# kmaninis/OSVOS-PyTorch

Measured on AMD Instinct MI355X. Metric: frames/sec (fwd+bwd) OSVOS-VGG16 854x480 per GPU; mask IoU vs ref, higher is better.
Workload: dtype f32 (3x bf16-split operands on MFMA, f32 accumulate); 1 GPU; 854x480 batch=1 online fine-tune loop (train_online.py), fused-head loss, nAveGrad=5, SGD 8-group, fp32x3, frame resident in HBM; global_batch=1, parallelism=dp1, grad_allreduce=none, rccl_ranks_seen=1

## Files before the change

osvos-pytorch_amd/csrc/wgrad_f32x3.hip:

```cpp
#include "common.h"
#include "kernels.h"
#include "h2split.h"

namespace {

typedef __bf16 bf16x8_t __attribute__((ext_vector_type(8)));
typedef __bf16 bf16x2_t __attribute__((ext_vector_type(2)));
typedef unsigned int u32x4 __attribute__((ext_vector_type(4)));
typedef short s16x4 __attribute__((ext_vector_type(4)));
typedef short s16x8 __attribute__((ext_vector_type(8)));
typedef __attribute__((address_space(3))) s16x4 lds_s16x4;

constexpr int PW = 16;

template <int PH_, int WAVES_, int S16_ = 0>
struct G3 {
  static constexpr int PH = PH_, WAVES = WAVES_, NT = 64 * WAVES_, S16 = S16_;
  static constexpr int BCO = S16_ ? 32 : 16 * WAVES_;
  static constexpr int BCI = S16_ ? 128 : 64;
  static constexpr int XOCT = BCI / 8;
  static constexpr int DYP = BCO * 2 + 64, XP = BCI * 2 + 64;
  static constexpr int PPIX = PW * PH, HW_ = PW + 2, XPIX = (PH + 2) * HW_;
  static constexpr int DY_B = PPIX * DYP, X_B = XPIX * XP;
  static constexpr int DOCT = BCO / 8;
  static constexpr int DY_ITEMS = PPIX * DOCT, X_ITEMS = XPIX * XOCT;
  static constexpr int DPG = NT / DOCT, XPG = NT / XOCT;
  static constexpr int NDY = (DY_ITEMS + NT - 1) / NT, NX = (X_ITEMS + NT - 1) / NT, NIT = NDY + NX;
  static constexpr int NST = 3 * PH;
  static constexpr int NB = WAVES_ == 8 ? 1 : 2;
  static constexpr size_t LDS = (size_t)3 * (DY_B + X_B);
  static_assert(NIT <= NST, "one staged item per stage must cover the patch");
  static_assert(LDS <= 160 * 1024, "tiles exceed the LDS of a CU");
};

struct W3Args {
  const void* x;
  const void* dy;
  float* slab;
  float* bslab;
  int N, H, W, Cin_s, Cout, Cout_s;
  int npx, npy, npatches, per_split, nco_t, nci_t;
  int map;
};

__device__ inline unsigned cvt2w(float a, float b) {
  bf16x2_t h;
  h[0] = (__bf16)a;
  h[1] = (__bf16)b;
  return __builtin_bit_cast(unsigned, h);
}
__device__ inline void split2w(float a, float b, unsigned& p0, unsigned& p1, unsigned& p2) {
  p0 = cvt2w(a, b);
  float ra = a - __uint_as_float(p0 << 16), rb = b - __uint_as_float(p0 & 0xffff0000u);
  p1 = cvt2w(ra, rb);
  ra -= __uint_as_float(p1 << 16);
  rb -= __uint_as_float(p1 & 0xffff0000u);
  p2 = cvt2w(ra, rb);
}
__device__ inline void split8w(const u32x4& lo, const u32x4& hi, u32x4& p0, u32x4& p1, u32x4& p2) {
  const f32x4 a = __builtin_bit_cast(f32x4, lo), b = __builtin_bit_cast(f32x4, hi);
  unsigned q0[4], q1[4], q2[4];
  split2w(a[0], a[1], q0[0], q1[0], q2[0]);
  split2w(a[2], a[3], q0[1], q1[1], q2[1]);
  split2w(b[0], b[1], q0[2], q1[2], q2[2]);
  split2w(b[2], b[3], q0[3], q1[3], q2[3]);
  p0 = u32x4{q0[0], q0[1], q0[2], q0[3]};
  p1 = u32x4{q1[0], q1[1], q1[2], q1[3]};
  p2 = u32x4{q2[0], q2[1], q2[2], q2[3]};
}

template <int NDS, int NVM, int NM = 18, int I = 0>
__device__ __forceinline__ void stage_groups() {
  if constexpr (I < NM) {
    __builtin_amdgcn_sched_group_barrier(0x008, 1, 0);
    constexpr int nds = (NDS * (I + 1)) / NM - (NDS * I) / NM, nvm = (NVM * (I + 1)) / NM - (NVM * I) / NM;
    if constexpr (nds > 0) __builtin_amdgcn_sched_group_barrier(0x100, nds, 0);
    if constexpr (nvm > 0) __builtin_amdgcn_sched_group_barrier(0x020, nvm, 0);
    __builtin_amdgcn_sched_group_barrier(0x006, 3, 0);
    stage_groups<NDS, NVM, NM, I + 1>();
  }
}

template <int PH, int WAVES, int S16 = 0, int ILV = 0, int NP = 3, int HP = 0, int OA = 0>
__global__ __launch_bounds__(64 * WAVES) void wgrad_f32x3_kernel(W3Args a) {
  static_assert(HP == 0 || NP == 2, "h2: two pieces");
  using G = G3<PH, WAVES, S16>;
  constexpr int NT = G::NT, BCO = G::BCO, BCI = G::BCI;
  extern __shared__ __attribute__((aligned(16))) char smem[];
  char* dYs = smem;
  char* Xs = smem + 3 * G::DY_B;
  const int tid = threadIdx.x, lane = tid & 63, wave = tid >> 6;
  const int wc = S16 ? 0 : wave >> 1, wi = S16 ? wave : wave & 1;
  constexpr unsigned OOB = 0x80000000u;

  int id = blockIdx.x;
  if (a.map == 1) id = (id & 7) * (gridDim.x >> 3) + (id >> 3);
  const int cit = id % a.nci_t;
  id /= a.nci_t;
  const int cot = id % a.nco_t;
  const int split = id / a.nco_t;
  const int co0 = cot * BCO, ci0 = cit * BCI;
  const int p_begin = split * a.per_split, p_end = min(p_begin + a.per_split, a.npatches);

  const int doct = tid % G::DOCT, dpg = tid / G::DOCT;
  const int xoct = tid % G::XOCT, xpg = tid / G::XOCT;
  const bool dy_ch_ok = co0 + 8 * doct < a.Cout, x_ch_ok = ci0 + 8 * xoct < a.Cin_s;
  u32x4 rdy[G::NDY][2], rx[G::NX][2];
  float bsum[8] = {0.f, 0.f, 0.f, 0.f, 0.f, 0.f, 0.f, 0.f};
  const bool want_bias = a.bslab != nullptr && cit == 0;
  const int img_dy_bytes = a.H * a.W * a.Cout_s * 4, img_x_bytes = a.H * a.W * a.Cin_s * 4;

  constexpr int DEADCOL = 0x40000000;
  unsigned dy_inv[G::NDY], x_inv[G::NX];
  unsigned dy_col[G::NDY], x_col[G::NX];
  if constexpr (OA == 0) {
#pragma unroll
    for (int it = 0; it < G::NDY; ++it) {
      const int p = dpg + G::DPG * it, py = p / PW, pxx = p - py * PW;
      const bool ok = dy_ch_ok && (G::DY_ITEMS % NT == 0 || p < G::PPIX);
      dy_inv[it] = (unsigned)(((py * a.W + pxx) * a.Cout_s + co0 + 8 * doct) * 4);
      dy_col[it] = (unsigned)(ok ? pxx : DEADCOL);
    }
#pragma unroll
    for (int j = 0; j < G::NX; ++j) {
      const int hp = xpg + G::XPG * j, hy = hp / G::HW_, hx = hp - hy * G::HW_;
      const bool ok = x_ch_ok && hp < G::XPIX;
      x_inv[j] = (unsigned)((((hy - 1) * a.W + hx - 1) * a.Cin_s + ci0 + 8 * xoct) * 4);
      x_col[j] = (unsigned)(ok ? hx - 1 : DEADCOL);
    }
  }

  struct Patch { __amdgpu_buffer_rsrc_t drs, xrs; int x0, y0; unsigned dorg, xorg; };
  auto locate = [&](int p, bool live) -> Patch {
    const int px = p % a.npx;
    int t = p / a.npx;
    const int py = t % a.npy;
    const int n = live ? t / a.npy : 0;
    Patch q;
    q.x0 = live ? px * PW : 0x40000000;
    q.y0 = py * PH;
    const unsigned org = (unsigned)(q.y0 * a.W + (live ? px * PW : 0));
    q.dorg = org * (unsigned)a.Cout_s * 4u;
    q.xorg = org * (unsigned)a.Cin_s * 4u;
    q.drs = __builtin_amdgcn_make_buffer_rsrc(const_cast<char*>(reinterpret_cast<const char*>(a.dy)) + (size_t)n * img_dy_bytes, 0, img_dy_bytes, 0x00020000);
    q.xrs = __builtin_amdgcn_make_buffer_rsrc(const_cast<char*>(reinterpret_cast<const char*>(a.x)) + (size_t)n * img_x_bytes, 0, img_x_bytes, 0x00020000);
    return q;
  };
  auto issue = [&](const Patch& q, int it) {
    if (it < G::NDY) {
      unsigned off;
      if constexpr (OA == 0) {
        off = (unsigned)q.x0 + dy_col[it] < (unsigned)a.W ? q.dorg + dy_inv[it] : OOB;
      } else {
        const int p = dpg + G::DPG * it, py = p / PW, pxx = p - py * PW;
        const bool ok = dy_ch_ok && (G::DY_ITEMS % NT == 0 || p < G::PPIX) && q.x0 + pxx < a.W;
        off = ok ? (unsigned)((((q.y0 + py) * a.W + q.x0 + pxx) * a.Cout_s + co0 + 8 * doct) * 4) : OOB;
      }
      rdy[it][0] = __builtin_amdgcn_raw_buffer_load_b128(q.drs, off, 0, 0);
      rdy[it][1] = __builtin_amdgcn_raw_buffer_load_b128(q.drs, off + 16u, 0, 0);
    } else if (it < G::NIT) {
      const int j = it - G::NDY;
      unsigned off;
      if constexpr (OA == 0) {
        off = (unsigned)q.x0 + x_col[j] < (unsigned)a.W ? q.xorg + x_inv[j] : OOB;
      } else {
        const int hp = xpg + G::XPG * j, hy = hp / G::HW_, hx = hp - hy * G::HW_;
        const bool ok = x_ch_ok && hp < G::XPIX && (unsigned)(q.x0 - 1 + hx) < (unsigned)a.W;
        off = ok ? (unsigned)((((q.y0 - 1 + hy) * a.W + q.x0 - 1 + hx) * a.Cin_s + ci0 + 8 * xoct) * 4) : OOB;
      }
      rx[j][0] = __builtin_amdgcn_raw_buffer_load_b128(q.xrs, off, 0, 0);
      rx[j][1] = __builtin_amdgcn_raw_buffer_load_b128(q.xrs, off + 16u, 0, 0);
    }
  };
  int h2_ed = kH2NoScale, h2_ex = kH2NoScale;
  float h2_sd = 1.f, h2_sx = 1.f;
  unsigned* const h2_mx = reinterpret_cast<unsigned*>(smem + G::LDS - 128);
  static_assert(HP == 0 || (G::X_B >= 128 && WAVES <= 8), "h2: exchange slots");
  auto store_patch = [&]() {
#pragma unroll
    for (int i = 0; i < G::NDY; ++i) {
      u32x4 p0, p1, p2;
      if (want_bias) {
        const f32x4 lo = __builtin_bit_cast(f32x4, rdy[i][0]), hi = __builtin_bit_cast(f32x4, rdy[i][1]);
#pragma unroll
        for (int c = 0; c < 4; ++c) { bsum[c] += lo[c]; bsum[4 + c] += hi[c]; }
      }
      if constexpr (HP != 0) h2_split8(rdy[i][0], rdy[i][1], h2_sd, p0, p1);
      else split8w(rdy[i][0], rdy[i][1], p0, p1, p2);
      const int p = dpg + G::DPG * i;
      if (G::DY_ITEMS % NT == 0 || p < G::PPIX) {
        char* d = dYs + p * G::DYP + doct * 16;
        *reinterpret_cast<u32x4*>(d) = p0;
        *reinterpret_cast<u32x4*>(d + G::DY_B) = p1;
        if constexpr (NP == 3) *reinterpret_cast<u32x4*>(d + 2 * G::DY_B) = p2;
      }
    }
#pragma unroll
    for (int j = 0; j < G::NX; ++j) {
      u32x4 p0, p1, p2;
      if constexpr (HP != 0) h2_split8(rx[j][0], rx[j][1], h2_sx, p0, p1);
      else split8w(rx[j][0], rx[j][1], p0, p1, p2);
      const int hp = xpg + G::XPG * j;
      if (G::X_ITEMS % NT == 0 || hp < G::XPIX) {
        char* d = Xs + hp * G::XP + xoct * 16;
        *reinterpret_cast<u32x4*>(d) = p0;
        *reinterpret_cast<u32x4*>(d + G::X_B) = p1;
        if constexpr (NP == 3) *reinterpret_cast<u32x4*>(d + 2 * G::X_B) = p2;
      }
    }
  };

  f32x16 acc[9];
#pragma unroll
  for (int t = 0; t < 9; ++t)
#pragma unroll
    for (int r = 0; r < 16; ++r) acc[t][r] = 0.f;

  const int fi = lane & 15, fg = (lane >> 4) & 1, lh = lane >> 5;
  const char* a_base = dYs + (8 * lh + (fi >> 2)) * G::DYP + (32 * wc + 16 * fg + 4 * (fi & 3)) * 2;
  const char* b_base = Xs + (8 * lh + (fi >> 2)) * G::XP + (32 * wi + 16 * fg + 4 * (fi & 3)) * 2;
  auto tr8 = [&](const char* p, int pitch) -> s16x8 {
    const s16x4 lo = __builtin_amdgcn_ds_read_tr16_b64_v4i16((lds_s16x4*)(p));
    const s16x4 hi = __builtin_amdgcn_ds_read_tr16_b64_v4i16((lds_s16x4*)(p + 4 * pitch));
    return __builtin_shufflevector(lo, hi, 0, 1, 2, 3, 4, 5, 6, 7);
  };

  {
    const Patch q = locate(p_begin, p_begin < p_end);
#pragma unroll
    for (int it = 0; it < G::NIT; ++it) issue(q, it);
  }
  for (int p = p_begin; p < p_end; ++p) {
    if constexpr (HP != 0) {
      unsigned md = 0, mxx = 0;
#pragma unroll
      for (int i = 0; i < G::NDY; ++i) md = h2_amax8(rdy[i][0], rdy[i][1], md);
#pragma unroll
      for (int j = 0; j < G::NX; ++j) mxx = h2_amax8(rx[j][0], rx[j][1], mxx);
      md = h2_wave_max(md);
      mxx = h2_wave_max(mxx);
      if (lane == 0) { h2_mx[(p & 1) * 16 + wave] = md; h2_mx[(p & 1) * 16 + 8 + wave] = mxx; }
    }
    __syncthreads();
    if constexpr (HP != 0) {
      const uint4* q = reinterpret_cast<const uint4*>(h2_mx) + (p & 1) * 4;
      const uint4 d0 = q[0], d1 = q[1], x0 = q[2], x1 = q[3];
      unsigned md = max(max(d0.x, d0.y), max(d0.z, d0.w)), mxx = max(max(x0.x, x0.y), max(x0.z, x0.w));
      if (WAVES == 8) { md = max(md, max(max(d1.x, d1.y), max(d1.z, d1.w))); mxx = max(mxx, max(max(x1.x, x1.y), max(x1.z, x1.w))); }
      const int ed = h2_exp(__builtin_amdgcn_readfirstlane(md)), ex = h2_exp(__builtin_amdgcn_readfirstlane(mxx));
      const int nd = ed < h2_ed ? ed : h2_ed, nx_ = ex < h2_ex ? ex : h2_ex;
      if (nd != h2_ed || nx_ != h2_ex) {
        const int dl = (h2_ed == kH2NoScale ? 0 : nd - h2_ed) + (h2_ex == kH2NoScale ? 0 : nx_ - h2_ex);
        if (dl != 0) {
#pragma unroll
          for (int t = 0; t < 9; ++t)
#pragma unroll
            for (int r = 0; r < 16; ++r) acc[t][r] = __builtin_ldexpf(acc[t][r], dl);
        }
        h2_ed = nd; h2_ex = nx_;
        h2_sd = h2_pow2(nd); h2_sx = h2_pow2(nx_);
      }
    }
    store_patch();
    __syncthreads();
    const Patch nx = locate(p + 1, p + 1 < p_end);
    constexpr int NB = G::NB;
    s16x8 af[NB][3], bfr[NB][3][3];
    auto lda = [&](int ks) {
#pragma unroll
      for (int pc = 0; pc < NP; ++pc) af[ks & (NB - 1)][pc] = tr8(a_base + pc * G::DY_B + ks * PW * G::DYP, G::DYP);
    };
    auto ldb = [&](int st) {
      const int ks = st / 3, r = st % 3;
#pragma unroll
      for (int pc = 0; pc < NP; ++pc)
#pragma unroll
        for (int s = 0; s < 3; ++s) bfr[st & (NB - 1)][pc][s] = tr8(b_base + pc * G::X_B + ((ks + r) * G::HW_ + s) * G::XP, G::XP);
    };
    if constexpr (NB == 2) {
      lda(0);
      ldb(0);
    }
#pragma unroll
    for (int st = 0; st < G::NST; ++st) {
      const int ks = st / 3, r = st % 3;
      if constexpr (NB == 2) {
        if (st + 1 < G::NST) {
          if (r == 2) lda(ks + 1);
          ldb(st + 1);
        }
      } else {
        if (r == 0) lda(ks);
        ldb(st);
      }
      issue(nx, st);
      if constexpr (ILV == 0) __builtin_amdgcn_sched_barrier(0);
      constexpr int NPROD = NP == 3 ? 6 : 3;
      constexpr int PX[6] = {NP == 3 ? 2 : 1, 0, NP == 3 ? 1 : 0, 1, 0, 0};
      constexpr int PD[6] = {0, NP == 3 ? 2 : 1, NP == 3 ? 1 : 0, 0, 1, 0};
#pragma unroll
      for (int t = 0; t < NPROD; ++t)
#pragma unroll
        for (int s = 0; s < 3; ++s)
          if constexpr (HP != 0)
            acc[r * 3 + s] = __builtin_amdgcn_mfma_f32_32x32x16_f16(__builtin_bit_cast(f16x8_t, bfr[st & (NB - 1)][PX[t]][s]),
                                                                   __builtin_bit_cast(f16x8_t, af[ks & (NB - 1)][PD[t]]), acc[r * 3 + s], 0, 0, 0);
          else
            acc[r * 3 + s] = __builtin_amdgcn_mfma_f32_32x32x16_bf16(__builtin_bit_cast(bf16x8_t, bfr[st & (NB - 1)][PX[t]][s]),
                                                                    __builtin_bit_cast(bf16x8_t, af[ks & (NB - 1)][PD[t]]), acc[r * 3 + s], 0, 0, 0);
      if constexpr (ILV != 0) {
        constexpr int V = 2;
        const bool last = st + 1 >= G::NST, wide = r == 2, vm = st < G::NIT;
        constexpr int NM = 3 * NPROD, DN = 6 * NP, DW = 8 * NP;
        if (last) { if (vm) stage_groups<0, V, NM>(); else stage_groups<0, 0, NM>(); }
        else if (wide) { if (vm) stage_groups<DW, V, NM>(); else stage_groups<DW, 0, NM>(); }
        else { if (vm) stage_groups<DN, V, NM>(); else stage_groups<DN, 0, NM>(); }
      }
      __builtin_amdgcn_sched_barrier(0);
    }
  }
  __syncthreads();
  if constexpr (HP != 0) {
    const int dl = (h2_ed == kH2NoScale || h2_ex == kH2NoScale) ? 0 : -(h2_ed + h2_ex);
#pragma unroll
    for (int t = 0; t < 9; ++t)
#pragma unroll
      for (int r = 0; r < 16; ++r) acc[t][r] = __builtin_ldexpf(acc[t][r], dl);
  }

  {
    const int li = lane & 31;
    const size_t slab_elems = (size_t)9 * a.Cout * a.Cin_s;
    const __amdgpu_buffer_rsrc_t srs = __builtin_amdgcn_make_buffer_rsrc(a.slab + (size_t)split * slab_elems, 0, (int)(slab_elems * 4), 0x00020000);
    const int co = co0 + wc * 32 + li;
    const int cib = ci0 + wi * 32 + 4 * lh;
    const unsigned row = co < a.Cout ? (unsigned)(co * a.Cin_s) * 4u : OOB;
    const unsigned tap_stride = (unsigned)(a.Cout * a.Cin_s) * 4u;
#pragma unroll
    for (int t = 0; t < 9; ++t)
#pragma unroll
      for (int q = 0; q < 4; ++q) {
        const int ci = cib + 8 * q;
        const unsigned off = ci < a.Cin_s ? row + (unsigned)t * tap_stride + (unsigned)ci * 4u : OOB;
        const f32x4 v = {acc[t][4 * q], acc[t][4 * q + 1], acc[t][4 * q + 2], acc[t][4 * q + 3]};
        __builtin_amdgcn_raw_buffer_store_b128(__builtin_bit_cast(u32x4, v), srs, off, 0, 0);
      }
  }
  if (want_bias) {
    float* red = reinterpret_cast<float*>(smem);
#pragma unroll
    for (int c = 0; c < 8; ++c) red[dpg * BCO + doct * 8 + c] = bsum[c];
    __syncthreads();
    if (tid < BCO) {
      float sum = 0.f;
      for (int g = 0; g < G::DPG; ++g) sum += red[g * BCO + tid];
      if (co0 + tid < a.Cout) a.bslab[(size_t)split * a.Cout + co0 + tid] = sum;
    }
  }
}

struct W3Plan {
  int ph, waves, bco, nco_t, nci_t, npx, npy, npatches, nsplit, per_split;
  size_t slab_floats, bslab_floats;
};

W3Plan make_plan3(int N, int H, int W, int Cin_s, int Cout) {
  W3Plan p;
  if (Cout == 16) {
    p.waves = 4; p.bco = 32; p.ph = 4;
    p.nco_t = 1;
    p.nci_t = ceil_div(Cin_s, 128);
    p.npx = ceil_div(W, PW);
    p.npy = ceil_div(H, p.ph);
    p.npatches = N * p.npx * p.npy;
    int want = ceil_div(256, p.nci_t);
    const int max_split = p.npatches / 2 > 0 ? p.npatches / 2 : 1;
    if (want > max_split) want = max_split;
    p.per_split = ceil_div(p.npatches, want);
    p.nsplit = ceil_div(p.npatches, p.per_split);
    p.slab_floats = (size_t)p.nsplit * 9 * Cout * Cin_s;
    p.bslab_floats = (size_t)p.nsplit * Cout;
    return p;
  }
  p.waves = 4;
  p.bco = 16 * p.waves;
  p.ph = (ceil_div(H, 6) * 6 <= ceil_div(H, 4) * 4) ? 6 : 4;
  p.nco_t = ceil_div(Cout, p.bco);
  p.nci_t = ceil_div(Cin_s, 64);
  p.npx = ceil_div(W, PW);
  p.npy = ceil_div(H, p.ph);
  p.npatches = N * p.npx * p.npy;
  int want = ceil_div(256, p.nco_t * p.nci_t);
  const int max_split = p.npatches / 2 > 0 ? p.npatches / 2 : 1;
  if (want > max_split) want = max_split;
  if (want > 256) want = 256;
  p.per_split = ceil_div(p.npatches, want);
  p.nsplit = ceil_div(p.npatches, p.per_split);
  p.slab_floats = (size_t)p.nsplit * 9 * Cout * Cin_s;
  p.bslab_floats = (size_t)p.nsplit * Cout;
  return p;
}

int block_map3(long blocks) {
  OSVOS_ENV_INT(map_env, "OSVOS_WGRAD_MAP", 1);
  return (map_env == 1 && blocks % 8 == 0) ? 1 : 0;
}

template <int PH, int WAVES, int S16 = 0, int ILV = 0, int NP = 3, int HP = 0, int OA = 0>
int launch3(const W3Args& a, long blocks, hipStream_t stream) {
  constexpr size_t lds = G3<PH, WAVES, S16>::LDS;
  if (int rc = osvos_set_dyn_lds_once<&wgrad_f32x3_kernel<PH, WAVES, S16, ILV, NP, HP, OA>>(lds)) return rc;
  hipLaunchKernelGGL((wgrad_f32x3_kernel<PH, WAVES, S16, ILV, NP, HP, OA>), dim3((unsigned)blocks), dim3(64 * WAVES), lds, stream, a);
  OSVOS_LAUNCH_CHECK();
  return 0;
}

}

bool osvos_wgrad_f32x3_applicable(int Cin, int Cin_s, int Cout, int Cout_s) {
  return Cin == Cin_s && Cin_s % 64 == 0 && Cout % 64 == 0 && Cout_s % 4 == 0;
}
bool osvos_wgrad_f32x3_skinny_applicable(int Cin, int Cin_s, int Cout, int Cout_s) {
  return Cout == 16 && Cout_s == 16 && Cin == Cin_s && Cin_s % 128 == 0;
}

size_t osvos_wgrad_f32x3_ws_bytes(int N, int H, int W, int Cin_s, int Cout) {
  if (Cout == 16 && Cin_s % 128 == 0) {
    const W3Plan p = make_plan3(N, H, W, Cin_s, Cout);
    return align_up((p.slab_floats + p.bslab_floats) * sizeof(float), 256);
  }
  if (Cin_s % 64 != 0 || Cout % 64 != 0) return 0;
  const W3Plan p = make_plan3(N, H, W, Cin_s, Cout);
  return align_up((p.slab_floats + p.bslab_floats) * sizeof(float), 256);
}

int osvos_wgrad_f32x3_plan(int N, int H, int W, int Cin_s, int Cout, int* out) {
  OSVOS_ARG_CHECK(osvos_wgrad_f32x3_applicable(Cin_s, Cin_s, Cout, Cout) || osvos_wgrad_f32x3_skinny_applicable(Cin_s, Cin_s, Cout, Cout),
                  "wgrad_wide_plan: no f32x3 weight-gradient kernel for Cin %d Cout %d", Cin_s, Cout);
  const W3Plan p = make_plan3(N, H, W, Cin_s, Cout);
  const long blocks = (long)p.nsplit * p.nco_t * p.nci_t;
  out[0] = PW; out[1] = p.ph; out[2] = p.npx; out[3] = p.npy; out[4] = p.npatches; out[5] = p.per_split; out[6] = p.nsplit;
  out[7] = p.nco_t; out[8] = p.nci_t; out[9] = (int)blocks; out[10] = block_map3(blocks); out[11] = 0;
  return 0;
}

int osvos_conv3x3_wgrad_f32x3(const WgradCall& c) {
  float *const dw = c.dw, *const db = c.db;
  void* const ws = c.ws; hipStream_t stream = c.stream;
  const int N = c.N, H = c.H, W = c.W, Cin = c.Cin, Cin_s = c.Cin_s, Cout = c.Cout, Cout_s = c.Cout_s, accumulate = c.accumulate;
  OSVOS_ARG_CHECK(c.x && c.dy && ws && dw, "wgrad f32x3: null pointer");
  OSVOS_ARG_CHECK(N > 0 && H > 0 && W > 0, "wgrad f32x3: bad shape");
  const bool skinny = Cout == 16 && Cout_s == 16 && Cin == Cin_s && Cin_s % 128 == 0;
  OSVOS_ARG_CHECK(skinny || osvos_wgrad_f32x3_applicable(Cin, Cin_s, Cout, Cout_s),
                  "wgrad f32x3: unsupported shape (Cin %d/%d Cout %d/%d)", Cin, Cin_s, Cout, Cout_s);
  OSVOS_ARG_CHECK((long)H * W * Cin_s < (1L << 28) && (long)H * W * Cout_s < (1L << 28), "wgrad f32x3: image too large for 31-bit byte offsets");
  OSVOS_ARG_CHECK(!c.x_bf16 && !c.dy_bf16, "wgrad f32x3: fp32 tensors only");
  const W3Plan p = make_plan3(N, H, W, Cin_s, Cout);
  W3Args a;
  a.x = c.x; a.dy = c.dy;
  a.slab = reinterpret_cast<float*>(ws);
  a.bslab = db ? a.slab + p.slab_floats : nullptr;
  a.N = N; a.H = H; a.W = W; a.Cin_s = Cin_s; a.Cout = Cout; a.Cout_s = Cout_s;
  a.npx = p.npx; a.npy = p.npy; a.npatches = p.npatches; a.per_split = p.per_split; a.nco_t = p.nco_t; a.nci_t = p.nci_t;
  const long blocks = (long)p.nsplit * p.nco_t * p.nci_t;
  a.map = block_map3(blocks);
  if (c.phase != WGRAD_REDUCE) {
    const bool two = c.pieces == 2;
    const bool h2 = c.pieces == 22;
    OSVOS_ENV_INT(oldaddr_env, "OSVOS_WGRAD_X3_OLDADDR", 0);
    const bool oa = oldaddr_env == 1 && !h2;
    const int rc = oa  ? (two ? (skinny ? launch3<4, 4, 1, 1, 2, 0, 1>(a, blocks, stream)
                                        : (p.ph == 6 ? launch3<6, 4, 0, 1, 2, 0, 1>(a, blocks, stream) : launch3<4, 4, 0, 1, 2, 0, 1>(a, blocks, stream)))
                              : (skinny ? launch3<4, 4, 1, 1, 3, 0, 1>(a, blocks, stream)
                                        : (p.ph == 6 ? launch3<6, 4, 0, 1, 3, 0, 1>(a, blocks, stream) : launch3<4, 4, 0, 1, 3, 0, 1>(a, blocks, stream))))
                 : h2  ? (skinny ? launch3<4, 4, 1, 1, 2, 1>(a, blocks, stream)
                                 : (p.ph == 6 ? launch3<6, 4, 0, 1, 2, 1>(a, blocks, stream) : launch3<4, 4, 0, 1, 2, 1>(a, blocks, stream)))
                 : two ? (skinny ? launch3<4, 4, 1, 1, 2>(a, blocks, stream)
                                 : (p.ph == 6 ? launch3<6, 4, 0, 1, 2>(a, blocks, stream) : launch3<4, 4, 0, 1, 2>(a, blocks, stream)))
                       : (skinny ? launch3<4, 4, 1, 1>(a, blocks, stream)
                                 : (p.ph == 6 ? launch3<6, 4, 0, 1>(a, blocks, stream) : launch3<4, 4, 0, 1>(a, blocks, stream)));
    if (rc) return rc;
  }
  if (c.phase == WGRAD_PARTIALS) return 0;
  return osvos_wgrad_reduce_launch(a.slab, a.bslab, dw, db, p.nsplit, Cout, Cin, Cin_s, accumulate, stream);
}
```

Measured before the change: 248.9 frames/s.

## Walk wgrad f32x3 inner loop by X input rows instead of (dY row, tap) stages

Reorders the weight-gradient MFMA loop so that each X input row is gathered from LDS once and used by all dY rows that pair with it. The old walk reloaded the X row for every (dY row, tap row) stage. dY fragments now live in a four-deep register ring, and staging of the next patch is spread across rows. A new scheduling-group helper interleaves the LDS reads with the MFMAs. The aim is to cut LDS transpose-read traffic, at the cost of more registers; the old stage walk stays reachable through an environment variable.

```diff
diff --git a/osvos-pytorch_amd/csrc/wgrad_f32x3.hip b/osvos-pytorch_amd/csrc/wgrad_f32x3.hip
--- a/osvos-pytorch_amd/csrc/wgrad_f32x3.hip
+++ b/osvos-pytorch_amd/csrc/wgrad_f32x3.hip
@@ -1,6 +1,8 @@
 #include "common.h"
 #include "kernels.h"
 #include "h2split.h"
+#include <string.h>
+#include <utility>
 
 namespace {
 
@@ -27,9 +29,11 @@
   static constexpr int DPG = NT / DOCT, XPG = NT / XOCT;
   static constexpr int NDY = (DY_ITEMS + NT - 1) / NT, NX = (X_ITEMS + NT - 1) / NT, NIT = NDY + NX;
   static constexpr int NST = 3 * PH;
-  static constexpr int NB = WAVES_ == 8 ? 1 : 2;
+  static constexpr int NROW = PH + 2;
+  static constexpr int IPR = (NIT + NROW - 1) / NROW;
   static constexpr size_t LDS = (size_t)3 * (DY_B + X_B);
-  static_assert(NIT <= NST, "one staged item per stage must cover the patch");
+  static_assert(WAVES_ == 4, "one wave per SIMD: two X row sets and four dY sets in registers");
+  static_assert(NIT <= IPR * NROW && NIT <= NST, "the staged items of a patch must fit its rows (stage walk: its stages)");
   static_assert(LDS <= 160 * 1024, "tiles exceed the LDS of a CU");
 };
 
@@ -81,10 +85,66 @@
   }
 }
 
-template <int PH, int WAVES, int S16 = 0, int ILV = 0, int NP = 3, int HP = 0, int OA = 0>
+template <int PH, int NP>
+struct RowWalk {
+  static constexpr int NROW = PH + 2, NPROD = NP == 3 ? 6 : 3;
+  static constexpr bool pairs(int y, int r) { return y - r >= 0 && y - r < PH; }
+  static constexpr int mfmas(int y) {
+    int n = 0;
+    for (int r = 0; r < 3; ++r) n += pairs(y, r) ? 3 * NPROD : 0;
+    return n;
+  }
+  static constexpr int gathers(int y) { return y + 1 >= NROW ? 0 : 2 * NP * (3 + (y + 1 < PH ? 1 : 0)); }
+  static constexpr bool every_pair_once() {
+    for (int ks = 0; ks < PH; ++ks)
+      for (int r = 0; r < 3; ++r) {
+        int n = 0;
+        for (int y = 0; y < NROW; ++y) n += pairs(y, r) && y - r == ks;
+        if (n != 1) return false;
+      }
+    return true;
+  }
+  static constexpr int patch_mfmas() {
+    int n = 0;
+    for (int y = 0; y < NROW; ++y) n += mfmas(y);
+    return n;
+  }
+  static constexpr bool gathered_set_is_free() {
+    for (int y = 0; y + 1 < PH; ++y)
+      for (int r = 0; r < 3; ++r)
+        if (pairs(y, r) && ((y - r) & 3) == ((y + 1) & 3)) return false;
+    return true;
+  }
+};
+
+template <int NDS, int NVM, int NM, int I = 0>
+__device__ __forceinline__ void row_groups() {
+  if constexpr (I < NM) {
+    __builtin_amdgcn_sched_group_barrier(0x008, 1, 0);
+    constexpr int per = NDS + 8 <= NM ? 1 : 2, left = NDS - per * I;
+    static_assert(NDS <= 2 * NM, "more than two gathers per MFMA gap");
+    constexpr int nds = left <= 0 ? 0 : (left < per ? left : per), nvm = (NVM * (I + 1)) / NM - (NVM * I) / NM;
+    if constexpr (nds > 0) __builtin_amdgcn_sched_group_barrier(0x100, nds, 0);
+    if constexpr (nvm > 0) __builtin_amdgcn_sched_group_barrier(0x020, nvm, 0);
+    __builtin_amdgcn_sched_group_barrier(0x006, 3, 0);
+    row_groups<NDS, NVM, NM, I + 1>();
+  }
+}
+template <class F, int... Y>
+__device__ __forceinline__ void for_rows(F&& f, std::integer_sequence<int, Y...>) {
+  (f(std::integral_constant<int, Y>{}), ...);
+}
+
+template <int PH, int WAVES, int S16 = 0, int ILV = 0, int NP = 3, int HP = 0, int OA = 0, int SW = 0>
 __global__ __launch_bounds__(64 * WAVES) void wgrad_f32x3_kernel(W3Args a) {
   static_assert(HP == 0 || NP == 2, "h2: two pieces");
+  static_assert(SW == 0 || (NP == 3 && HP == 0 && OA == 0), "the stage walk is kept for the production three-piece forms only");
   using G = G3<PH, WAVES, S16>;
+  using RW = RowWalk<PH, NP>;
+  static_assert(RW::every_pair_once(), "every (dY row, tap row) pair exactly once per patch");
+  static_assert(RW::patch_mfmas() == 9 * RW::NPROD * PH && (NP != 3 || RW::patch_mfmas() == 18 * 3 * PH), "MFMAs of a patch: 18 (three pieces) per (dY row, tap row) pair, 3 PH pairs");
+  static_assert(RW::gathered_set_is_free(), "row y gathers dY set (y + 1) & 3 while its MFMAs read it");
+  static_assert(RW::NROW == G::NROW, "rows");
   constexpr int NT = G::NT, BCO = G::BCO, BCI = G::BCI;
   extern __shared__ __attribute__((aligned(16))) char smem[];
   char* dYs = smem;
@@ -264,59 +324,93 @@
     store_patch();
     __syncthreads();
     const Patch nx = locate(p + 1, p + 1 < p_end);
-    constexpr int NB = G::NB;
-    s16x8 af[NB][3], bfr[NB][3][3];
-    auto lda = [&](int ks) {
-#pragma unroll
-      for (int pc = 0; pc < NP; ++pc) af[ks & (NB - 1)][pc] = tr8(a_base + pc * G::DY_B + ks * PW * G::DYP, G::DYP);
-    };
-    auto ldb = [&](int st) {
-      const int ks = st / 3, r = st % 3;
-#pragma unroll
-      for (int pc = 0; pc < NP; ++pc)
-#pragma unroll
-        for (int s = 0; s < 3; ++s) bfr[st & (NB - 1)][pc][s] = tr8(b_base + pc * G::X_B + ((ks + r) * G::HW_ + s) * G::XP, G::XP);
-    };
-    if constexpr (NB == 2) {
+    constexpr int NPROD = RW::NPROD;
+    constexpr int PX[6] = {NP == 3 ? 2 : 1, 0, NP == 3 ? 1 : 0, 1, 0, 0};
+    constexpr int PD[6] = {0, NP == 3 ? 2 : 1, NP == 3 ? 1 : 0, 0, 1, 0};
+    if constexpr (SW == 0) {
+      s16x8 af[4][3], bfr[2][3][3];
+      auto lda = [&](int ks, int pc) { af[ks & 3][pc] = tr8(a_base + pc * G::DY_B + ks * PW * G::DYP, G::DYP); };
+      auto ldb = [&](int y, int pc) {
+#pragma unroll
+        for (int s = 2; s >= 0; --s) bfr[y & 1][pc][s] = tr8(b_base + pc * G::X_B + (y * G::HW_ + s) * G::XP, G::XP);
+      };
+#pragma unroll
+      for (int t = 0; t < NP; ++t) { lda(0, PD[t]); ldb(0, PX[t]); }
+      __builtin_amdgcn_sched_barrier(0);
+      for_rows([&](auto row) __attribute__((always_inline)) {
+        constexpr int y = decltype(row)::value;
+        if constexpr (y + 1 < G::NROW) {
+          constexpr bool dy_row = y + 1 < PH;
+#pragma unroll
+          for (int pc = 0; pc < NP; ++pc) {
+            if (pc != PX[0]) ldb(y + 1, pc);
+            if (dy_row && pc != PD[0]) lda(y + 1, pc);
+          }
+          ldb(y + 1, PX[0]);
+          if constexpr (dy_row) lda(y + 1, PD[0]);
+        }
+        constexpr int it0 = y * G::IPR, nit = it0 >= G::NIT ? 0 : (G::NIT - it0 < G::IPR ? G::NIT - it0 : G::IPR);
+#pragma unroll
+        for (int i = 0; i < nit; ++i) issue(nx, it0 + i);
+        if constexpr (ILV == 0) __builtin_amdgcn_sched_barrier(0);
+#pragma unroll
+        for (int t = 0; t < NPROD; ++t)
+#pragma unroll
+          for (int r = 0; r < 3; ++r)
+            if (RW::pairs(y, r)) {
+              const int ks = y - r;
+#pragma unroll
+              for (int s = 0; s < 3; ++s)
+                if constexpr (HP != 0)
+                  acc[r * 3 + s] = __builtin_amdgcn_mfma_f32_32x32x16_f16(__builtin_bit_cast(f16x8_t, bfr[y & 1][PX[t]][s]),
+                                                                         __builtin_bit_cast(f16x8_t, af[ks & 3][PD[t]]), acc[r * 3 + s], 0, 0, 0);
+                else
+                  acc[r * 3 + s] = __builtin_amdgcn_mfma_f32_32x32x16_bf16(__builtin_bit_cast(bf16x8_t, bfr[y & 1][PX[t]][s]),
+                                                                          __builtin_bit_cast(bf16x8_t, af[ks & 3][PD[t]]), acc[r * 3 + s], 0, 0, 0);
+            }
+        if constexpr (ILV != 0) row_groups<RW::gathers(y), 2 * nit, RW::mfmas(y)>();
+        __builtin_amdgcn_sched_barrier(0);
+      }, std::make_integer_sequence<int, G::NROW>{});
+    } else {
+      s16x8 af[2][3], bfr[2][3][3];
+      auto lda = [&](int ks) {
+#pragma unroll
+        for (int pc = 0; pc < NP; ++pc) af[ks & 1][pc] = tr8(a_base + pc * G::DY_B + ks * PW * G::DYP, G::DYP);
+      };
+      auto ldb = [&](int st) {
+        const int ks = st / 3, r = st % 3;
+#pragma unroll
+        for (int pc = 0; pc < NP; ++pc)
+#pragma unroll
+          for (int s = 0; s < 3; ++s) bfr[st & 1][pc][s] = tr8(b_base + pc * G::X_B + ((ks + r) * G::HW_ + s) * G::XP, G::XP);
+      };
       lda(0);
       ldb(0);
-    }
-#pragma unroll
-    for (int st = 0; st < G::NST; ++st) {
-      const int ks = st / 3, r = st % 3;
-      if constexpr (NB == 2) {
+#pragma unroll
+      for (int st = 0; st < G::NST; ++st) {
+        const int ks = st / 3, r = st % 3;
         if (st + 1 < G::NST) {
           if (r == 2) lda(ks + 1);
           ldb(st + 1);
         }
-      } else {
-        if (r == 0) lda(ks);
-        ldb(st);
-      }
-      issue(nx, st);
-      if constexpr (ILV == 0) __builtin_amdgcn_sched_barrier(0);
-      constexpr int NPROD = NP == 3 ? 6 : 3;
-      constexpr int PX[6] = {NP == 3 ? 2 : 1, 0, NP == 3 ? 1 : 0, 1, 0, 0};
-      constexpr int PD[6] = {0, NP == 3 ? 2 : 1, NP == 3 ? 1 : 0, 0, 1, 0};
-#pragma unroll
-      for (int t = 0; t < NPROD; ++t)
-#pragma unroll
-        for (int s = 0; s < 3; ++s)
-          if constexpr (HP != 0)
-            acc[r * 3 + s] = __builtin_amdgcn_mfma_f32_32x32x16_f16(__builtin_bit_cast(f16x8_t, bfr[st & (NB - 1)][PX[t]][s]),
-                                                                   __builtin_bit_cast(f16x8_t, af[ks & (NB - 1)][PD[t]]), acc[r * 3 + s], 0, 0, 0);
-          else
-            acc[r * 3 + s] = __builtin_amdgcn_mfma_f32_32x32x16_bf16(__builtin_bit_cast(bf16x8_t, bfr[st & (NB - 1)][PX[t]][s]),
-                                                                    __builtin_bit_cast(bf16x8_t, af[ks & (NB - 1)][PD[t]]), acc[r * 3 + s], 0, 0, 0);
-      if constexpr (ILV != 0) {
-        constexpr int V = 2;
-        const bool last = st + 1 >= G::NST, wide = r == 2, vm = st < G::NIT;
-        constexpr int NM = 3 * NPROD, DN = 6 * NP, DW = 8 * NP;
-        if (last) { if (vm) stage_groups<0, V, NM>(); else stage_groups<0, 0, NM>(); }
-        else if (wide) { if (vm) stage_groups<DW, V, NM>(); else stage_groups<DW, 0, NM>(); }
-        else { if (vm) stage_groups<DN, V, NM>(); else stage_groups<DN, 0, NM>(); }
-      }
-      __builtin_amdgcn_sched_barrier(0);
+        issue(nx, st);
+        if constexpr (ILV == 0) __builtin_amdgcn_sched_barrier(0);
+#pragma unroll
+        for (int t = 0; t < NPROD; ++t)
+#pragma unroll
+          for (int s = 0; s < 3; ++s)
+            acc[r * 3 + s] = __builtin_amdgcn_mfma_f32_32x32x16_bf16(__builtin_bit_cast(bf16x8_t, bfr[st & 1][PX[t]][s]),
+                                                                    __builtin_bit_cast(bf16x8_t, af[ks & 1][PD[t]]), acc[r * 3 + s], 0, 0, 0);
+        if constexpr (ILV != 0) {
+          constexpr int V = 2;
+          const bool last = st + 1 >= G::NST, wide = r == 2, vm = st < G::NIT;
+          constexpr int NM = 3 * NPROD, DN = 6 * NP, DW = 8 * NP;
+          if (last) { if (vm) stage_groups<0, V, NM>(); else stage_groups<0, 0, NM>(); }
+          else if (wide) { if (vm) stage_groups<DW, V, NM>(); else stage_groups<DW, 0, NM>(); }
+          else { if (vm) stage_groups<DN, V, NM>(); else stage_groups<DN, 0, NM>(); }
+        }
+        __builtin_amdgcn_sched_barrier(0);
+      }
     }
   }
   __syncthreads();
@@ -406,11 +500,11 @@
   return (map_env == 1 && blocks % 8 == 0) ? 1 : 0;
 }
 
-template <int PH, int WAVES, int S16 = 0, int ILV = 0, int NP = 3, int HP = 0, int OA = 0>
+template <int PH, int WAVES, int S16 = 0, int ILV = 0, int NP = 3, int HP = 0, int OA = 0, int SW = 0>
 int launch3(const W3Args& a, long blocks, hipStream_t stream) {
   constexpr size_t lds = G3<PH, WAVES, S16>::LDS;
-  if (int rc = osvos_set_dyn_lds_once<&wgrad_f32x3_kernel<PH, WAVES, S16, ILV, NP, HP, OA>>(lds)) return rc;
-  hipLaunchKernelGGL((wgrad_f32x3_kernel<PH, WAVES, S16, ILV, NP, HP, OA>), dim3((unsigned)blocks), dim3(64 * WAVES), lds, stream, a);
+  if (int rc = osvos_set_dyn_lds_once<&wgrad_f32x3_kernel<PH, WAVES, S16, ILV, NP, HP, OA, SW>>(lds)) return rc;
+  hipLaunchKernelGGL((wgrad_f32x3_kernel<PH, WAVES, S16, ILV, NP, HP, OA, SW>), dim3((unsigned)blocks), dim3(64 * WAVES), lds, stream, a);
   OSVOS_LAUNCH_CHECK();
   return 0;
 }
@@ -469,7 +563,11 @@
     const bool h2 = c.pieces == 22;
     OSVOS_ENV_INT(oldaddr_env, "OSVOS_WGRAD_X3_OLDADDR", 0);
     const bool oa = oldaddr_env == 1 && !h2;
-    const int rc = oa  ? (two ? (skinny ? launch3<4, 4, 1, 1, 2, 0, 1>(a, blocks, stream)
+    static const bool stage_env = [] { const char* e = getenv("OSVOS_WGRAD_X3_WALK"); return e && strcmp(e, "stage") == 0; }();
+    const bool sw = stage_env && !oa && !h2 && !two;
+    const int rc = sw  ? (skinny ? launch3<4, 4, 1, 1, 3, 0, 0, 1>(a, blocks, stream)
+                                 : (p.ph == 6 ? launch3<6, 4, 0, 1, 3, 0, 0, 1>(a, blocks, stream) : launch3<4, 4, 0, 1, 3, 0, 0, 1>(a, blocks, stream)))
+                 : oa  ? (two ? (skinny ? launch3<4, 4, 1, 1, 2, 0, 1>(a, blocks, stream)
                                         : (p.ph == 6 ? launch3<6, 4, 0, 1, 2, 0, 1>(a, blocks, stream) : launch3<4, 4, 0, 1, 2, 0, 1>(a, blocks, stream)))
                               : (skinny ? launch3<4, 4, 1, 1, 3, 0, 1>(a, blocks, stream)
                                         : (p.ph == 6 ? launch3<6, 4, 0, 1, 3, 0, 1>(a, blocks, stream) : launch3<4, 4, 0, 1, 3, 0, 1>(a, blocks, stream))))
```

After: 250.4 frames/s (median of 6 runs). Within noise of the previous version (+0.6%).
